# StephenNG59/ICP-symm

Hardware: AMD Instinct MI355X
Metric: icp_iterations_per_sec (higher is better)
Workload: dtype f32

## Files before the change

### icp-symm_amd/csrc/engine_loop.cpp

```cpp
#include "engine_internal.h"

extern "C" {

static int prepare_rejectors(symmicp_ctx *c, RejectArgs &r)
{
    Rejectors &j = c->rej;
    r = RejectArgs{};
    if (!pass_rejects(c)) return SYMMICP_OK;
    HIP_TRY(c, grow(j.keys, j.keys_cap, c->n_loc ? c->n_loc : 1));
    if (!j.ws) HIP_TRY(c, hipMalloc((void **)&j.ws, sizeof(uint32_t) * kRejectWsWords));
    r.keys = j.keys; r.ws = j.ws;
    r.host = reinterpret_cast<RejectRecord *>(c->h_sums_dev + kNSum + 1);
    r.rho = j.trim_frac; r.med_f2 = j.median() ? j.med_factor * j.med_factor : 0.0f;
    if (!pass_claims(c)) return SYMMICP_OK;
    HIP_TRY(c, grow(j.table, j.table_cap, Rejectors::table_words(c->n_t, pass_reciprocal(c))));
    r.table = j.table; r.n_t = c->n_t; r.order = c->src_order;
    r.claim = kClaimOneToOne;
    if (!pass_reciprocal(c)) return SYMMICP_OK;
    if (!j.src_ix.valid) {
        const double t0 = now_s();
        if (int st = build_reverse_index(c, c->src0, c->n_loc, c->src_order, j.src_ix)) return st;
        j.src_ix_builds++;
        if (c->sw.debug_host) {
            std::fprintf(stderr, "[symmicp host] source index: %u points, %zu bytes in its arena (+%zu allocations beside it), built in %.3f ms\n", c->n_loc,
// ... 223 lines not shown
    if (pass_rejects(c)) return false;
    if (c->cfg.mode == SYMMICP_MODE_COLOR) return false;
    if (c->cfg.host_loop) return false;
    if (c->external_exchange || c->shm.slots) return false;
    if (c->timing == 2 || c->ix.dbg) return false;
    if (!mode_device_solves(c->cfg.mode)) return false;
    if (c->n_loc == 0 && !c->comm) return false;
    if (c->host_passes_since_bailout < 2) return false;
    const bool incr = resolved_apply(c->cfg) == SYMMICP_APPLY_INCREMENTAL;
    if (c->cfg.corr == SYMMICP_CORR_IDENTITY) return true;
    if (c->cfg.corr == SYMMICP_CORR_TREE)
        return !incr && c->last_list_len >= 0 && c->last_list_len <= (c->sw.no_loop_stragglers ? 0ll : (long long)kLoopListLimit) && c->last_uncertified >= 0 &&
               c->last_uncertified <= (long long)(loop_scan_limit(c->n_s_total) / (c->last_list_len > 0 ? 2 : 1)) && c->cert && !c->sw.no_cert;
    return false;
}

static constexpr int kListBlocks = 8;
static constexpr int kEvSampleStride = 4;
static int run_batch(symmicp_ctx *c, int want, float *diffs_before, int *n_done, bool *small_step)
{
    *n_done = 0;
    *small_step = false;
    if (want > symmicp_ctx::kRing - 1) want = symmicp_ctx::kRing - 1;
    if (want <= 0) return SYMMICP_OK;
    const bool incr = resolved_apply(c->cfg) == SYMMICP_APPLY_INCREMENTAL;
    const bool tree = c->cfg.corr == SYMMICP_CORR_TREE;
    LoopConfig lc{};
    lc.mode = c->cfg.mode; lc.fixed_iters = c->cfg.fixed_iters; lc.max_iters = c->iters + want; lc.incremental = incr ? 1 : 0; lc.tree = tree ? 1 : 0;
    lc.diff_threshold = c->cfg.diff_threshold; lc.eps_rotation = c->cfg.eps_rotation; lc.eps_translation = c->cfg.eps_translation;
    lc.nrm_w = (c->cfg.mode == SYMMICP_MODE_QUIRKS) ? 1.0f : 0.0f;
    for (int k = 0; k < 3; k++) lc.pivot[k] = c->pivot[k];
    lc.uncertified_limit = 4 * loop_scan_limit(c->n_s_total);
    const bool no_stage = c->sw.no_loop_stragglers;
    bool stragglers = tree && c->last_list_len > 0 && !no_stage;
    lc.list_limit = kLoopListLimit;
    const int cert_mode = (tree && c->cert && !c->sw.no_cert && !c->cert_pass_failed) ? c->sw.cert_pass : 0;
    if (cert_mode == 2) stragglers = false;
    bool cert_chunk = false;
    uint8_t pass_kernel[symmicp_ctx::kRing] = {};
    if (lc.max_iters > c->cfg.max_iters) lc.max_iters = c->cfg.max_iters;
    const int it0 = c->iters;
    const long long list0 = c->last_list_len, scans0 = c->last_scans;
    LoopState ls{};
    std::memcpy(ls.X, c->X, sizeof(ls.X));
    for (int k = 0; k < 12; k++) ls.Xapply.m[k] = c->X[k];
    ls.Xapply.nrm_w = lc.nrm_w;
    ls.iters = it0;
    *c->h_loop = ls;
    symmicp_sums last0{};
    if (c->loop_log_on) {
        last0 = c->last;
        c->h_ring[it0 % symmicp_ctx::kRing].solved = 0;
    }
    HIP_TRY(c, hipMemcpyAsync(c->d_loop, c->h_loop, sizeof(LoopState), hipMemcpyHostToDevice, c->stream));
    PassArgs a{};
    fill_pass_args(c, a, RejectArgs{}, c->X, incr, incr, false);
    a.loop = c->d_loop;
    int blocks;
    bool vec4 = false;
    if (tree) {
        const int fb = c->sw.fused_blocks;
        const int tiles = (int)((c->n_loc + kPassThreads - 1) / kPassThreads);
        blocks = tiles < fb ? tiles : fb;
        if (blocks < 1) blocks = 1;
    } else {
        vec4 = (c->n_loc % 4 == 0) && (c->n_t % 4 == 0) && (c->src_off % 4 == 0);
        const int id_cap = c->sw.id_blocks;
        const int nb = (int)(((vec4 ? c->n_loc / 4 : c->n_loc) + kPassThreads - 1) / kPassThreads);
        blocks = nb < id_cap ? (nb > 0 ? nb : 1) : id_cap;
    }
    const int fused_blocks_full = blocks;
    c->pass_blocks = blocks;
    uint32_t *counters = tree ? c->wl_count : nullptr;
    const bool timed_run = c->timing == 1 || c->timing == 3;
    const int ev_stride = c->timing == 3 ? kEvSampleStride : 1;
    if (timed_run && c->ev_used + want > symmicp_ctx::kEvRing) flush_events(c);
    const bool one_piece = lc.fixed_iters && !(lc.eps_rotation > 0.f && lc.eps_translation > 0.f);
    int enq = 0, n_stage = 0;
    constexpr int kCertHeads = 3;
    int heads_left = (one_piece && !stragglers && cert_mode == 1 && c->sw.cert_head > 0) ? kCertHeads : 0;
    auto plan_chunk = [&](long long list_len, long long scans, int left, int prev) -> int {
        cert_chunk = cert_mode == 2 || (cert_mode == 1 && !stragglers && list_len == 0 && scans == 0);
        if (stragglers) return 4;
        if (!one_piece) return prev ? 2 * prev : 4;
        if (!cert_chunk && heads_left > 0 && left > c->sw.cert_head) { heads_left--; return c->sw.cert_head; }
        return left;
    };
    int chunk = plan_chunk(c->last_list_len, c->last_scans, want, 0);
    bool first_chunk = true;
    while (enq < want) {
        const int nq = (want - enq < chunk) ? want - enq : chunk;
        const int it_before = first_chunk ? it0 : c->h_loop->iters;
        const int ev_used0 = c->ev_used;
        const int fused_blocks = (stragglers && fused_blocks_full + kListBlocks > 512) ? 512 - kListBlocks : fused_blocks_full;
        blocks = fused_blocks + (stragglers ? kListBlocks : 0);
        a.partial_cols = stragglers ? (uint32_t)blocks : 0u;
        a.partial_col0 = (uint32_t)fused_blocks;
        lc.walk_in_loop = stragglers ? 1 : 0;
        if (first_chunk) launch_reduce_solve(c->partials, blocks, c->d_sums, 2, c->d_loop, lc, c->h_ring_dev, symmicp_ctx::kRing, counters, c->stream);
        for (int p = 0; p < nq; p++) {
            hipEvent_t *ev = nullptr;
            if (timed_run && (enq + p) % ev_stride == 0 && c->ev_used < symmicp_ctx::kEvRing) {
                ev = c->ev + c->ev_used * symmicp_ctx::kEvPer;
                c->ev_split[c->ev_used] = 1;
                c->ev_weight[c->ev_used] = 1;
                hipEventRecord(ev[0], c->stream);
            }
            if (tree) {
                pass_kernel[(it_before + 1 + p) % symmicp_ctx::kRing] = cert_chunk ? 1 : 0;
                if (cert_chunk) launch_pass_certified(a, c->ix, c->wl, fused_blocks, c->stream);
                else launch_pass_fused(a, c->ix, c->wl, fused_blocks, c->stream);
                if (stragglers) launch_loop_stragglers(a, c->ix, c->wl, kListBlocks, c->sw.tune, c->stream);
            }
            else launch_pass_identity(a, c->tgt, blocks, vec4, c->stream);
            if (ev) { hipEventRecord(ev[4], c->stream); c->ev_used++; }
            if (c->comm || blocks > 512) {
                launch_final_reduce(c->partials, blocks, c->d_sums, nullptr, c->ticket, 0ull, counters, 0, c->stream);
                if (c->comm) {
                    if (ev) { hipEventRecord(ev[6], c->stream); c->ev_coll[c->ev_used - 1] = 1; }
                    int r = g_rccl.AllReduce(c->d_sums, c->d_sums, kNSum, kNcclFloat64, kNcclSum, c->comm, c->stream);
                    if (r != 0) {
                        (void)hipStreamSynchronize(c->stream);
                        c->begun = false;
                        c->ev_used = 0;
                        return fail(c, SYMMICP_ERR_COMM, std::string("ncclAllReduce: ") + (g_rccl.GetErrorString ? g_rccl.GetErrorString(r) : "?"));
                    }
                    if (ev) hipEventRecord(ev[7], c->stream);
                }
                launch_reduce_solve(c->partials, blocks, c->d_sums, 1, c->d_loop, lc, c->h_ring_dev, symmicp_ctx::kRing, counters, c->stream);
            } else {
                launch_reduce_solve(c->partials, blocks, c->d_sums, 0, c->d_loop, lc, c->h_ring_dev, symmicp_ctx::kRing, counters, c->stream);
            }
        }
        const unsigned long long seq = ++c->batch_seq;
        launch_loop_end(c->d_loop, c->h_loop_dev, c->h_done_dev, seq, c->stream);
        if (int st = wait_for_word(c, c->h_done, seq, 60.0, "batch finished without publishing its end flag")) return st;
        enq += nq;
        first_chunk = false;
        const int ran = (c->h_loop->iters - it_before) + (c->h_loop->reason == LOOP_REDO_PASS ? 1 : 0);
        if (timed_run && ran >= 0) {
            int sampled_ran = 0;
            for (int p = 0; p < ran && p < nq; p++) {
                if ((enq - nq + p) % ev_stride != 0) continue;
                if (ev_used0 + sampled_ran < symmicp_ctx::kEvRing) {
                    const int left = (ran < nq ? ran : nq) - p;
                    c->ev_weight[ev_used0 + sampled_ran] = left < ev_stride ? left : ev_stride;
                }
                sampled_ran++;
            }
            if (ev_used0 + sampled_ran < c->ev_used) c->ev_used = ev_used0 + sampled_ran;
        }
        if (stragglers) n_stage += c->h_loop->iters - it_before;
        if (c->h_loop->stop) break;
        if (tree && !no_stage) {
            stragglers = false;
            for (int k = it_before + 1; k <= c->h_loop->iters; k++) stragglers = stragglers || c->h_ring[k % symmicp_ctx::kRing].list_len > 0;
        }
        if (cert_mode == 2) stragglers = false;
        const LoopRecord &lr = c->h_ring[c->h_loop->iters % symmicp_ctx::kRing];
        chunk = plan_chunk(lr.list_len, lr.reserved, want - enq, chunk);
    }
    const LoopState &hl = *c->h_loop;
    const int it1 = hl.iters;
    if (it1 < it0 || it1 > it0 + want) return fail(c, SYMMICP_ERR_HIP, "device loop state out of range");
    for (int k = it0; k < it1; k++) diffs_before[k - it0] = (k == it0) ? (float)c->last.s[33] : (float)c->h_ring[k % symmicp_ctx::kRing].sums[33];
    if (it1 > it0) {
        std::memcpy(c->last.s, c->h_ring[it1 % symmicp_ctx::kRing].sums, sizeof(double) * kNSum);
        std::memcpy(c->X, c->h_ring[(it1 - 1) % symmicp_ctx::kRing].X, sizeof(float) * 16);
        c->st.passes += it1 - it0;
        c->st.loop_passes += it1 - it0;
        c->st.loop_straggler_passes += n_stage;
    }
    if (c->loop_log_on) {
        for (int k = it0; k <= it1; k++) {
            const LoopRecord &r = c->h_ring[k % symmicp_ctx::kRing];
            symmicp_loop_log_entry e{};
            std::memcpy(e.sums, k == it0 ? last0.s : r.sums, sizeof(e.sums));
            std::memcpy(e.increment, r.increment, sizeof(e.increment));
            std::memcpy(e.X, r.X, sizeof(e.X));
            e.rcond = r.rcond; e.iter = k; e.status = r.status; e.solved = r.solved; e.list_len = k == it0 ? 0 : r.list_len;
            e.reason = hl.reason; e.batch = c->loop_log_batches;
            e.reserved = k == it0 ? 0 : pass_kernel[k % symmicp_ctx::kRing];
            if (k == it1 && hl.reason == LOOP_REDO_PASS && pass_kernel[(it1 + 1) % symmicp_ctx::kRing]) e.reserved |= 0x100;
            if (!e.solved) { std::memset(e.increment, 0, sizeof(e.increment)); std::memset(e.X, 0, sizeof(e.X)); e.rcond = 0.f; e.status = -1; }
            c->loop_log.push_back(e);
        }
        c->loop_log_batches++;
    }
// ... 240 lines not shown
    HIP_TRY(c, hipSetDevice(c->device));
    const size_t b_sums = sizeof(symmicp_sums) * n, b_f3 = sizeof(float) * 3 * n, b_16 = sizeof(float) * 16 * n;
    const size_t o_piv = b_sums, o_xin = o_piv + 16, o_st = o_xin + b_16, o_pb = o_st + 4 * n, o_qb = o_pb + b_f3, o_a = o_qb + b_f3, o_t = o_a + b_f3,
                 o_rc = o_t + b_f3, o_out = o_rc + 4 * n, o_xo = o_out + b_16, total = o_xo + b_16;
    char *d = nullptr;
    HIP_TRY(c, hipMalloc((void **)&d, total));
    float piv[4] = {0.f, 0.f, 0.f, 0.f};
    if (pivot) for (int k = 0; k < 3; k++) piv[k] = pivot[k];
    int st = SYMMICP_OK;
    if (hipMemcpy(d, sums, b_sums, hipMemcpyHostToDevice) != hipSuccess || hipMemcpy(d + o_piv, piv, 16, hipMemcpyHostToDevice) != hipSuccess ||
        (X_in16 && hipMemcpy(d + o_xin, X_in16, b_16, hipMemcpyHostToDevice) != hipSuccess))
        st = fail(c, SYMMICP_ERR_HIP, "probe: upload");
    if (st == SYMMICP_OK) {
        launch_solve_probe(mode, exact_rc, (const symmicp_sums *)d, (int)n, (const float *)(d + o_piv), X_in16 ? (const float *)(d + o_xin) : nullptr,
                           (int32_t *)(d + o_st), (float *)(d + o_pb), (float *)(d + o_qb), (float *)(d + o_a), (float *)(d + o_t), (float *)(d + o_rc),
                           (float *)(d + o_out), (float *)(d + o_xo), c->stream);
        if (hipGetLastError() != hipSuccess || hipStreamSynchronize(c->stream) != hipSuccess) st = fail(c, SYMMICP_ERR_HIP, "probe: kernel");
    }
    if (st == SYMMICP_OK) {
        const struct { size_t off, bytes; void *dst; } back[] = {{o_st, 4 * n, status}, {o_pb, b_f3, pbar}, {o_qb, b_f3, qbar}, {o_a, b_f3, a}, {o_t, b_f3, t},
                                                              {o_rc, 4 * n, rcond}, {o_out, b_16, out16}, {o_xo, X_in16 ? b_16 : 0, X_out16}};
        for (const auto &b : back)
            if (b.bytes && hipMemcpy(b.dst, d + b.off, b.bytes, hipMemcpyDeviceToHost) != hipSuccess) { st = fail(c, SYMMICP_ERR_HIP, "probe: read back"); break; }
    }
    (void)hipFree(d);
    return st;
}

int symmicp_ctx_loop_solve(symmicp_ctx *c, const symmicp_sums *sums, const float pivot[3], const float X_in16[16], const int32_t in_i[6], const float in_f[3],
                           int32_t state_out[4], float X_out16[16], float Xapply_out12[12], float ring_inc16[16], float ring_X16[16], float *ring_rcond,
                           int32_t ring_i2[2])
{
    if (!c) return SYMMICP_ERR_ARG;
    if (!sums || !X_in16 || !in_i || !in_f || !state_out || !X_out16 || !Xapply_out12 || !ring_inc16 || !ring_X16 || !ring_rcond || !ring_i2)
        return fail(c, SYMMICP_ERR_ARG, "loop_solve: bad arguments");
    const int mode = in_i[0];
    if (!mode_device_solves(mode)) return fail(c, SYMMICP_ERR_ARG, "loop_solve: QUIRKS, PAPER, PLANE or GICP");
    HIP_TRY(c, hipSetDevice(c->device));
    LoopConfig lc{};
    lc.mode = mode; lc.fixed_iters = in_i[1]; lc.max_iters = in_i[2]; lc.incremental = in_i[5] ? 1 : 0; lc.tree = 0;
    lc.diff_threshold = in_f[0]; lc.eps_rotation = in_f[1]; lc.eps_translation = in_f[2];
    lc.nrm_w = (mode == SYMMICP_MODE_QUIRKS) ? 1.0f : 0.0f;
    for (int k = 0; k < 3; k++) lc.pivot[k] = pivot ? pivot[k] : 0.f;
    LoopState ls{};
    std::memcpy(ls.X, X_in16, sizeof(ls.X));
    for (int k = 0; k < 12; k++) ls.Xapply.m[k] = X_in16[k];
    ls.Xapply.nrm_w = lc.nrm_w;
    ls.iters = in_i[3];
    ls.small_step = in_i[4];
    char *d = nullptr;
    const size_t o_loop = 512, o_ring = o_loop + ((sizeof(LoopState) + 255) & ~(size_t)255), total = o_ring + sizeof(LoopRecord);
    HIP_TRY(c, hipMalloc((void **)&d, total));
    int st = SYMMICP_OK;
    if (hipMemcpy(d, sums, sizeof(symmicp_sums), hipMemcpyHostToDevice) != hipSuccess || hipMemcpy(d + o_loop, &ls, sizeof(ls), hipMemcpyHostToDevice) != hipSuccess ||
        hipMemset(d + o_ring, 0xFF, sizeof(LoopRecord)) != hipSuccess)
        st = fail(c, SYMMICP_ERR_HIP, "loop_solve: upload");
    if (st == SYMMICP_OK) {
        launch_reduce_solve(nullptr, 0, (double *)d, 2, (LoopState *)(d + o_loop), lc, (LoopRecord *)(d + o_ring), 1, nullptr, c->stream);
        if (hipGetLastError() != hipSuccess || hipStreamSynchronize(c->stream) != hipSuccess) st = fail(c, SYMMICP_ERR_HIP, "loop_solve: kernel");
    }
    LoopState lo{};
    LoopRecord r{};
    if (st == SYMMICP_OK && (hipMemcpy(&lo, d + o_loop, sizeof(lo), hipMemcpyDeviceToHost) != hipSuccess ||
                             hipMemcpy(&r, d + o_ring, sizeof(r), hipMemcpyDeviceToHost) != hipSuccess))
        st = fail(c, SYMMICP_ERR_HIP, "loop_solve: read back");
    (void)hipFree(d);
    if (st != SYMMICP_OK) return st;
    state_out[0] = lo.stop; state_out[1] = lo.reason; state_out[2] = lo.iters; state_out[3] = lo.small_step;
    std::memcpy(X_out16, lo.X, sizeof(lo.X));
    std::memcpy(Xapply_out12, lo.Xapply.m, sizeof(lo.Xapply.m));
    std::memcpy(ring_inc16, r.increment, sizeof(r.increment));
    std::memcpy(ring_X16, r.X, sizeof(r.X));
    std::memcpy(ring_rcond, &r.rcond, sizeof(float));
    ring_i2[0] = r.status; ring_i2[1] = r.solved;
    return SYMMICP_OK;
}

int symmicp_set_loop_log(symmicp_ctx *c, int on)
{
    if (!c) return SYMMICP_ERR_ARG;
    c->loop_log_on = on != 0;
    if (!c->loop_log_on) { c->loop_log.clear(); c->loop_log.shrink_to_fit(); }
    return SYMMICP_OK;
}

int symmicp_get_loop_log(const symmicp_ctx *c, symmicp_loop_log_entry *out, size_t cap, size_t *count)
{
    if (!c || !count) return SYMMICP_ERR_ARG;
    *count = c->loop_log.size();
    if (out) std::memcpy(out, c->loop_log.data(), sizeof(symmicp_loop_log_entry) * std::min(cap, c->loop_log.size()));
    return SYMMICP_OK;
}

}
```

### icp-symm_amd/csrc/kernels_pass.hip

```cpp
#include <cstdlib>
#include <type_traits>
#include "symmicp_internal.h"
#include "device_common.h"
#include "oct_walk.h"
#include "solve_core.h"
#include "robust_loss.h"
#include "pass_rows.h"
#pragma clang fp contract(off)

namespace symmicp {

template <int NA>
__device__ __forceinline__ void acc_block_reduce_store(AccN<NA> &a, double *partials, uint32_t col)
{
    __shared__ double red[(kPassThreads / 64) * kNSum];
    acc_wave_reduce(a, red + (threadIdx.x >> 6) * kNSum);
    __syncthreads();
    if (threadIdx.x < kNSum) {
        double s = 0.0;
        if (threadIdx.x < NA) {
#pragma unroll
            for (int w = 0; w < kPassThreads / 64; w++) s += red[w * kNSum + threadIdx.x];
        }
        partials[(size_t)col * kNSum + threadIdx.x] = s;
// ... 1118 lines not shown

__global__ __launch_bounds__(256) void k_final_reduce(const double *__restrict__ partials, int nblocks,
                                                      double *out_dev, double *out_mapped, uint32_t *ticket,
                                                      unsigned long long seq, uint32_t *counters_to_clear, int keep_nonempty)
{
    __shared__ double red[256];
    const int k = blockIdx.x, t = threadIdx.x;
    double s = 0.0;
    for (int j = t; j < nblocks; j += 256) s += partials[(size_t)j * kNSum + k];
    red[t] = s;
    __syncthreads();
#pragma unroll
    for (int off = 128; off > 0; off >>= 1) {
        if (t < off) red[t] += red[t + off];
        __syncthreads();
    }
    __shared__ int last;
    if (t == 0) {
        out_dev[k] = red[0];
        if (out_mapped) out_mapped[k] = red[0];
        __threadfence_system();
        last = (atomicAdd(ticket, 1u) == gridDim.x - 1);
    }
    __syncthreads();
    if (last) {
        if (counters_to_clear) {
            __shared__ uint32_t s_len;
            if (t < 64) {
                uint32_t len, searched, dropped, scans;
                read_list_words(counters_to_clear, t, len, searched, dropped, scans);
                if (t == 0) {
                    s_len = len;
                    const double lenw = (double)len + (dropped ? kListDropped : 0.0), srw = (double)searched + (double)scans * kScanUnit;
                    out_dev[kNSum - 1] = lenw; out_dev[kNSum - 2] = srw;
                    if (out_mapped) { out_mapped[kNSum - 1] = lenw; out_mapped[kNSum - 2] = srw; }
                }
            }
            __syncthreads();
            if (t < 2) counters_to_clear[t * kShards * kShardStride + 2] = 0;
            if (t < kShards) { counters_to_clear[t * kShardStride + 1] = 0; counters_to_clear[t * kShardStride + 3] = 0; }
            if (!(keep_nonempty && s_len > 0u))
                for (int c = t; c < 2 * kShards; c += 256) counters_to_clear[c * kShardStride] = 0;
        }
        if (t == 0) {
            *ticket = 0;
            if (out_mapped) {
                __threadfence_system();
                reinterpret_cast<volatile unsigned long long *>(out_mapped)[kNSum] = seq;
            }
        }
    }
}

template <bool REDUCE>
__global__ __launch_bounds__(512) void k_reduce_solve(const double *__restrict__ partials, int nblocks, double *out_dev, int solve_only, LoopState *loop,
                                                       LoopConfig cfg, LoopRecord *ring, int ring_len, uint32_t *counters_to_clear)
{
    __shared__ double s_sum[kNSum];
    __shared__ uint32_t s_len, s_unc, s_scan;
    const int t = threadIdx.x, lane = t & 63, wave = t >> 6;
#ifdef RS_STAMPS
    const unsigned long long ts0 = __builtin_amdgcn_s_memrealtime();
#endif
    const LoopState ls = *loop;
    uint32_t cw0 = 0, cw1 = 0, cw2 = 0, cw3 = 0;
    const bool want_counters = !solve_only && REDUCE && counters_to_clear && t < 64;
    if (want_counters) {
        cw0 = counters_to_clear[t * kShardStride]; cw1 = counters_to_clear[t * kShardStride + 1];
        cw2 = (t < 2) ? counters_to_clear[t * kShards * kShardStride + 2] : 0u;
        cw3 = counters_to_clear[t * kShardStride + 3];
    }
    __shared__ double s_part[8][kNSum];
    double accw = 0.0;
    if (!solve_only && REDUCE && lane < kNSum) {
        if (nblocks <= 512) {
            double c[64];
#pragma unroll
            for (int j = 0; j < 64; j++) { const int b = wave + 8 * j; c[j] = (b < nblocks) ? partials[(size_t)b * kNSum + lane] : 0.0; }
#pragma unroll
            for (int j = 0; j < 64; j++) accw += c[j];
        } else {
            for (int b = wave; b < nblocks; b += 8) accw += partials[(size_t)b * kNSum + lane];
        }
    }
    double rec = 0.0;
    if ((solve_only || !REDUCE) && t < kNSum) rec = out_dev[t];
    if (ls.stop) return;
#ifdef RS_STAMPS
    const unsigned long long tsA = __builtin_amdgcn_s_memrealtime();
#endif
    if (t == 0) { s_len = 0; s_unc = 0; s_scan = 0; }
    if (!solve_only && REDUCE) {
        if (lane < kNSum) s_part[wave][lane] = accw;
        __syncthreads();
        if (t < kNSum) {
            double x = 0.0;
#pragma unroll
            for (int w = 0; w < 8; w++) x += s_part[w][t];
            s_sum[t] = (t < kNAccW) ? x : 0.0;
        }
    } else if (t < kNSum) s_sum[t] = rec;
    __syncthreads();
    if (!solve_only && counters_to_clear) {
        if (REDUCE) {
            if (t < 64) {
#pragma unroll
                for (int off = 32; off > 0; off >>= 1) {
                    cw0 += (uint32_t)__shfl_xor((int)cw0, off, 64);
                    cw1 += (uint32_t)__shfl_xor((int)cw1, off, 64);
                    cw2 += (uint32_t)__shfl_xor((int)cw2, off, 64);
                    cw3 += (uint32_t)__shfl_xor((int)cw3, off, 64);
                }
                if (t == 0) { s_len = cw2 ? 0xFFFFFFFFu : cw0; s_unc = cw1; s_scan = cw1 > cw3 ? cw1 - cw3 : 0u; }
            }
            if (t < kShards) { counters_to_clear[t * kShardStride + 1] = 0; counters_to_clear[t * kShardStride + 3] = 0; }
            for (int c = t; c < 2 * kShards; c += 512) counters_to_clear[c * kShardStride] = 0;
        } else if (t == 0) {
            s_len = (s_sum[kNSum - 1] >= kListDropped) ? 0xFFFFFFFFu : (uint32_t)s_sum[kNSum - 1];
            const double sr = s_sum[kNSum - 2], sc = floor(sr / kScanUnit);
            s_unc = (uint32_t)(sr - sc * kScanUnit); s_scan = (uint32_t)sc;
        }
    }
    __syncthreads();
#ifdef RS_STAMPS
    const unsigned long long ts1 = __builtin_amdgcn_s_memrealtime();
#endif
    int it = ls.iters;
    if (!solve_only) {
        const uint32_t len = s_len, unc = s_unc, scans = s_scan;
        if (cfg.tree && len > 0u && (!cfg.walk_in_loop || len == 0xFFFFFFFFu)) { if (t == 0) { loop->stop = 1; loop->reason = LOOP_REDO_PASS; } return; }
        it += 1;
        LoopRecord &r = ring[it % ring_len];
        if (t < kNSum) { const double v = (t >= kNAccW) ? 0.0 : s_sum[t]; r.sums[t] = v; if (REDUCE) out_dev[t] = v; }
        if (t == 0) {
            loop->iters = it;
            r.solved = 0;
            r.pad = (int32_t)unc;
            r.list_len = (int32_t)len; r.reserved = (int32_t)scans;
        }
        if (cfg.tree && (unc > cfg.uncertified_limit || (cfg.walk_in_loop && len > cfg.list_limit))) { if (t == 0) { loop->stop = 1; loop->reason = LOOP_SLOW; } return; }
    }
    if (t != 0) return;
    const float diff = (float)s_sum[33];
    if (ls.small_step || !((cfg.fixed_iters || diff > cfg.diff_threshold) && it < cfg.max_iters)) {
        loop->stop = 1; loop->reason = LOOP_DONE;
        return;
    }
    symmicp_sums S;
    for (int k = 0; k < kNSum; k++) S.s[k] = (k >= kNAccW) ? 0.0 : s_sum[k];
    float pbar[3], qbar[3], av[3], tv[3], rc = 0.f, Xi[16];
    const int st = solve::solve_mode(cfg.mode, S, cfg.pivot, pbar, qbar, av, tv, &rc, Xi, false);
    if (st != SYMMICP_OK || !(rc > 1e-6f)) { loop->stop = 1; loop->reason = LOOP_HOST_SOLVE; return; }
#ifdef RS_STAMPS
    const unsigned long long ts2 = __builtin_amdgcn_s_memrealtime();
#endif
    float Xn[16];
    solve::mat4_mul(Xi, ls.X, Xn);
    for (int k = 0; k < 16; k++) loop->X[k] = Xn[k];
    const float *ap = cfg.incremental ? Xi : Xn;
    for (int k = 0; k < 12; k++) loop->Xapply.m[k] = ap[k];
    loop->Xapply.nrm_w = cfg.nrm_w;
    LoopRecord &r = ring[it % ring_len];
    for (int k = 0; k < 16; k++) { r.increment[k] = Xi[k]; r.X[k] = Xn[k]; }
    r.rcond = rc; r.status = st; r.solved = 1;
#ifdef RS_STAMPS2
    r.sums[37] = partials[(size_t)8191 * kNSum]; r.sums[38] = partials[(size_t)8191 * kNSum + 1]; r.sums[39] = partials[(size_t)8191 * kNSum + 2];
#elif defined(RS_STAMPS)
    r.sums[37] = (double)(ts1 - ts0) + 1e-4 * (double)(tsA - ts0); r.sums[38] = (double)(ts2 - ts1); r.sums[39] = (double)(__builtin_amdgcn_s_memrealtime() - ts2);
#endif
    if (cfg.eps_rotation > 0.f && cfg.eps_translation > 0.f && !cfg.fixed_iters) {
        const double tr = ((double)Xi[0] + Xi[5] + Xi[10] - 1.0) * 0.5;
        const double ang = acos(tr > 1.0 ? 1.0 : (tr < -1.0 ? -1.0 : tr));
        const double tn = sqrt((double)Xi[3] * Xi[3] + (double)Xi[7] * Xi[7] + (double)Xi[11] * Xi[11]);
        if (ang < cfg.eps_rotation && tn < cfg.eps_translation) loop->small_step = 1;
    }
}

__global__ __launch_bounds__(64) void k_solve_probe(int mode, int exact_rc, const symmicp_sums *__restrict__ sums, int n, const float *pivot,
                                                    const float *__restrict__ X_in, int32_t *status, float *pbar, float *qbar, float *a, float *t,
                                                    float *rcond, float *out16, float *X_out)
{
    const int i = blockIdx.x * blockDim.x + threadIdx.x;
    if (i >= n) return;
    const symmicp_sums S = sums[i];
    float pb[3] = {0.f, 0.f, 0.f}, qb[3] = {0.f, 0.f, 0.f}, av[3] = {0.f, 0.f, 0.f}, tv[3] = {0.f, 0.f, 0.f}, rc = 0.f, Xi[16], Xn[16];
    for (int k = 0; k < 16; k++) Xi[k] = 0.f;
    const bool ex = exact_rc != 0;
    const int st = solve::solve_mode(mode, S, pivot, pb, qb, av, tv, &rc, Xi, ex);
    status[i] = st;
    rcond[i] = rc;
    for (int k = 0; k < 3; k++) { pbar[3 * i + k] = pb[k]; qbar[3 * i + k] = qb[k]; a[3 * i + k] = av[k]; t[3 * i + k] = tv[k]; }
    for (int k = 0; k < 16; k++) out16[16 * (size_t)i + k] = Xi[k];
    if (X_in) {
        solve::mat4_mul(Xi, X_in + 16 * (size_t)i, Xn);
        for (int k = 0; k < 16; k++) X_out[16 * (size_t)i + k] = Xn[k];
    }
}

void launch_solve_probe(int mode, int exact_rc, const symmicp_sums *sums, int n, const float *pivot, const float *X_in, int32_t *status, float *pbar,
                        float *qbar, float *a, float *t, float *rcond, float *out16, float *X_out, hipStream_t s)
{
    if (n > 0) hipLaunchKernelGGL(k_solve_probe, dim3((n + 63) / 64), dim3(64), 0, s, mode, exact_rc, sums, n, pivot, X_in, status, pbar, qbar, a, t, rcond, out16, X_out);
}

__global__ __launch_bounds__(64) void k_loop_end(const LoopState *loop, LoopState *host_copy, unsigned long long *done_flag, unsigned long long seq)
{
    if (threadIdx.x == 0) {
        *host_copy = *loop;
        __threadfence_system();
        *reinterpret_cast<volatile unsigned long long *>(done_flag) = seq;
    }
}

__global__ __launch_bounds__(64) void k_publish(const double *__restrict__ sums_dev, double *out_mapped, unsigned long long seq)
{
    if (threadIdx.x < kNSum) out_mapped[threadIdx.x] = sums_dev[threadIdx.x];
    __threadfence_system();
    __syncthreads();
    if (threadIdx.x == 0) {
        __threadfence_system();
        reinterpret_cast<volatile unsigned long long *>(out_mapped)[kNSum] = seq;
    }
}

__global__ __launch_bounds__(kPassThreads) void k_nn_brute(CloudSoA src, uint32_t n_s, Affine X,
                                                          const float4 *__restrict__ tq, uint32_t n_t,
                                                          uint32_t tiles_per_split, unsigned long long *best64)
{
    __shared__ float4 tile[kBruteTile];
    float px[kBruteQ], py[kBruteQ], pz[kBruteQ], bd[kBruteQ];
    uint32_t bj[kBruteQ];
    const uint32_t q0 = blockIdx.x * (kPassThreads * kBruteQ) + threadIdx.x;
#pragma unroll
    for (int k = 0; k < kBruteQ; k++) {
        uint32_t i = q0 + k * kPassThreads;
        float x = 0.f, y = 0.f, z = 0.f;
        if (i < n_s) { x = src.x[i]; y = src.y[i]; z = src.z[i]; }
        px[k] = xf_row(X.m + 0, x, y, z, 1.0f); py[k] = xf_row(X.m + 4, x, y, z, 1.0f); pz[k] = xf_row(X.m + 8, x, y, z, 1.0f);
        bd[k] = __int_as_float(0x7f800000); bj[k] = 0xFFFFFFFFu;
    }
    const uint32_t tile0 = blockIdx.y * tiles_per_split;
    const uint32_t ntiles = (n_t + kBruteTile - 1) / kBruteTile;
    const uint32_t tile1 = min(tile0 + tiles_per_split, ntiles);
    for (uint32_t t = tile0; t < tile1; t++) {
        const uint32_t base = t * kBruteTile;
        __syncthreads();
#pragma unroll
        for (int k = 0; k < kBruteTile / kPassThreads; k++) {
            uint32_t j = base + k * kPassThreads + threadIdx.x;
            tile[k * kPassThreads + threadIdx.x] = (j < n_t) ? tq[j] : make_float4(__int_as_float(0x7fc00000), 0.f, 0.f, 0.f);
        }
        __syncthreads();
#pragma unroll 4
        for (int j = 0; j < kBruteTile; j++) {
            float4 q = tile[j];
#pragma unroll
            for (int k = 0; k < kBruteQ; k++) {
                float d2 = dist2(px[k], py[k], pz[k], q.x, q.y, q.z);
                if (d2 < bd[k]) { bd[k] = d2; bj[k] = base + j; }
            }
        }
    }
#pragma unroll
    for (int k = 0; k < kBruteQ; k++) {
// ... 119 lines not shown
            uint32_t qshift = nb >= 3072u ? 8u : (nb >= 1536u ? 7u : 6u);
            if (tune.cells_queries == 64u) qshift = 6u; else if (tune.cells_queries == 128u) qshift = 7u; else if (tune.cells_queries == 256u) qshift = 8u;
            const uint32_t nq = (a.n + (1u << qshift) - 1u) >> qshift;
            const uint32_t nbc = ((nq + 8u * chunk - 1u) / (8u * chunk)) * (8u * chunk);
            if (a.make_hood) hipLaunchKernelGGL(k_search_cells<true>, dim3(nbc), dim3(kPassThreads), 0, s, a, ix, wl, chunk, qshift);
            else hipLaunchKernelGGL(k_search_cells<false>, dim3(nbc), dim3(kPassThreads), 0, s, a, ix, wl, chunk, qshift);
        }
    }
    if (ev) hipEventRecord(ev[1], s);
    if (ev) hipEventRecord(ev[2], s);
    if (stage != 1 && nbp) {
        if (walk_blocks == 0 || walk_blocks > walk_blocks_full(wl)) walk_blocks = walk_blocks_full(wl);
        const uint32_t wmm = a.pos_prev ? wave_mode_max : 0u;
        if (a.budget_walk) {
            const uint32_t budget = tune.walk_budget;
            hipLaunchKernelGGL(k_search_walk<true>, dim3(walk_blocks), dim3(kWalkThreads), 0, s, a, ix, wl, wl.work, wmm, budget);
            hipLaunchKernelGGL(k_search_walk<false>, dim3(8192), dim3(kWalkThreads), 0, s, a, ix, wl, wl.retry, 0xFFFFFFFFu, 0xFFFFFFFFu);
        } else {
            hipLaunchKernelGGL(k_search_walk<false>, dim3(walk_blocks), dim3(kWalkThreads), 0, s, a, ix, wl, wl.work, wmm, 0xFFFFFFFFu);
        }
    }
    if (ev) hipEventRecord(ev[3], s);
    launch_accumulate(a, ix.tn, acc_blocks, s);
    if (ev) hipEventRecord(ev[4], s);
}

void launch_final_reduce(const double *partials, int blocks, double *out_dev, double *out_host_mapped, uint32_t *ticket,
                         unsigned long long seq, uint32_t *counters_to_clear, int keep_nonempty, hipStream_t s)
{
    hipLaunchKernelGGL(k_final_reduce, dim3(kNSum), dim3(256), 0, s, partials, blocks, out_dev, out_host_mapped, ticket, seq,
                       counters_to_clear, keep_nonempty);
}

void launch_pass_fused(const PassArgs &a, const TargetIndex &ix, const WorkLists &wl, int blocks, hipStream_t s)
{
    with_instantiation(a, [&](auto W, auto OBJ) { hipLaunchKernelGGL((k_pass_fused<true, W, OBJ>), dim3(blocks), dim3(kPassThreads), 0, s, a, ix, wl); });
}

void launch_pass_certified(const PassArgs &a, const TargetIndex &ix, const WorkLists &wl, int blocks, hipStream_t s)
{
    with_instantiation(a, [&](auto W, auto OBJ) { hipLaunchKernelGGL((k_pass_certified<W, OBJ>), dim3(blocks), dim3(kPassThreads), 0, s, a, ix, wl); });
}

void launch_loop_stragglers(const PassArgs &a, const TargetIndex &ix, const WorkLists &wl, int list_blocks, const PassTuning &tune, hipStream_t s)
{
    const uint32_t wave_mode_max = tune.wave_mode_max;
    hipLaunchKernelGGL(k_search_walk<false>, dim3(512), dim3(kWalkThreads), 0, s, a, ix, wl, wl.work, wave_mode_max, 0xFFFFFFFFu);
    with_instantiation(a, [&](auto W, auto OBJ) {
        hipLaunchKernelGGL((k_accumulate_list<W, OBJ>), dim3(list_blocks), dim3(kPassThreads), 0, s, a, ix.tn, wl.work);
    });
}

void launch_reduce_solve(const double *partials, int blocks, double *out_dev, int mode, LoopState *loop, LoopConfig cfg, LoopRecord *ring, int ring_len,
                         uint32_t *counters_to_clear, hipStream_t s)
{
    if (mode == 0) hipLaunchKernelGGL(k_reduce_solve<true>, dim3(1), dim3(512), 0, s, partials, blocks, out_dev, 0, loop, cfg, ring, ring_len, counters_to_clear);
    else hipLaunchKernelGGL(k_reduce_solve<false>, dim3(1), dim3(512), 0, s, partials, blocks, out_dev, mode == 2 ? 1 : 0, loop, cfg, ring, ring_len, counters_to_clear);
}

void launch_loop_end(const LoopState *loop, LoopState *host_copy, unsigned long long *done_flag, unsigned long long seq, hipStream_t s)
{
    hipLaunchKernelGGL(k_loop_end, dim3(1), dim3(64), 0, s, loop, host_copy, done_flag, seq);
}

void launch_publish(const double *sums_dev, double *out_host_mapped, unsigned long long seq, hipStream_t s)
{
    hipLaunchKernelGGL(k_publish, dim3(1), dim3(64), 0, s, sums_dev, out_host_mapped, seq);
}

void launch_nn_brute(const CloudSoA &src, uint32_t n_s, const Affine &X, const float4 *tq, uint32_t n_t,
                     unsigned long long *best64, hipStream_t s)
{
    const uint32_t qblocks = (n_s + kPassThreads * kBruteQ - 1) / (kPassThreads * kBruteQ);
    const uint32_t ntiles = (n_t + kBruteTile - 1) / kBruteTile;
    uint32_t splits = 1;
    if (qblocks < 2048) splits = (2048 + qblocks - 1) / qblocks;
    if (splits > ntiles) splits = ntiles;
    if (splits < 1) splits = 1;
    if (splits > 65535) splits = 65535;
    const uint32_t tiles_per_split = (ntiles + splits - 1) / splits;
    splits = (ntiles + tiles_per_split - 1) / tiles_per_split;
    hipMemsetAsync(best64, 0xFF, sizeof(unsigned long long) * (size_t)n_s, s);
    hipLaunchKernelGGL(k_nn_brute, dim3(qblocks, splits), dim3(kPassThreads), 0, s, src, n_s, X, tq, n_t, tiles_per_split, best64);
}

}
```

### icp-symm_amd/csrc/symmicp_internal.h

```cpp
#pragma once
#include <hip/hip_runtime.h>
#include <stdint.h>
#include <stddef.h>
#include "symmicp.h"

namespace symmicp {

constexpr int kNSum = SYMMICP_NSUM;
constexpr int kNAcc = 37;
constexpr int kNAccW = 38;
constexpr double kListDropped = 4294967296.0;
constexpr double kScanUnit = 4294967296.0;
constexpr int kLeaf = 8;
constexpr int kFan = 8;
constexpr int kMaxTreeLevels = 12;
constexpr int kMortonBits = 10;
constexpr int kPassThreads = 256;
constexpr int kBruteTile = 1024;
constexpr int kBruteQ = 4;

constexpr bool mode_device_solves(int mode)
{
    return mode == SYMMICP_MODE_QUIRKS || mode == SYMMICP_MODE_PAPER || mode == SYMMICP_MODE_PLANE || mode == SYMMICP_MODE_GICP;
}
// ... 147 lines not shown
    RejectArgs rej;
    const float4 *tgt_color;
    const float *src_int;
    float color_lam, color_om;
};
static_assert(sizeof(PassArgs) == 432 && offsetof(PassArgs, rej) == 344 && offsetof(PassArgs, tgt_color) == 408 && offsetof(PassArgs, src_int) == 416,
              "PassArgs keeps its layout");
__host__ __device__ inline bool pass_rejects(const PassArgs &a) { return a.rej.keys != nullptr; }

struct PassTuning {
    uint32_t wave_mode_max = 20000u;
    uint32_t cells_chunk = 16u;
    uint32_t cells_queries = 0u;
    uint32_t walk_budget = 160u;
};

constexpr int kBatchThreads = 512;
constexpr int kBatchQ = 4;
constexpr int kBatchChunk = kBatchThreads * kBatchQ;
constexpr int kBatchTile = SYMMICP_BATCH_MAX_POINTS;
constexpr int kBatchMerge = 1024;
__host__ __device__ constexpr uint32_t batch_splits(uint32_t n) { return n <= 256u ? 8u : n <= 512u ? 4u : n <= 1024u ? 2u : 1u; }
static_assert(kBatchThreads / 8 >= 64 && (kBatchThreads / 2) * kBatchQ == kBatchMerge, "a split is at least one wave; two splits cover kBatchMerge rows");
struct BatchProblem {
    uint32_t src_first, src_count, tgt_first, tgt_count;
    float pivot[3];
    uint32_t slot;
};
struct BatchArgs {
    const float *src_xyz, *src_nrm, *tgt_xyz, *tgt_nrm;
    const BatchProblem *problems;
    const float *guess;
    symmicp_batch_result *out;
    float *trace_X;
    double *trace_sums;
    int32_t mode, max_iters, fixed_iters;
    float diff_threshold, max_d2, min_ndot, eps_rotation, eps_translation;
};
void launch_batch_align(const BatchArgs &a, uint32_t n_problems, hipStream_t s);

void launch_pass_identity(const PassArgs &a, CloudSoA tgt, int blocks, bool vec4_ok, hipStream_t s);
void launch_pass_indexed(const PassArgs &a, const float4 *tn , int blocks, hipStream_t s);
void launch_pass_tree_split(const PassArgs &a, const TargetIndex &ix, const WorkLists &wl, int acc_blocks, uint32_t walk_blocks,
                            int stage, int compact_blocks, const PassTuning &tune, hipStream_t s, hipEvent_t *ev);
void launch_pass_tree_first(const PassArgs &a, const TargetIndex &ix, const WorkLists &wl, int acc_blocks, hipStream_t s, hipEvent_t *ev);
uint32_t walk_blocks_full(const WorkLists &wl);
uint32_t shard_capacity(uint32_t n_points);
void launch_final_reduce(const double *partials, int blocks, double *out_dev, double *out_host_mapped, uint32_t *ticket,
                         unsigned long long seq, uint32_t *counters_to_clear, int keep_nonempty, hipStream_t s);
void launch_pass_fused(const PassArgs &a, const TargetIndex &ix, const WorkLists &wl, int blocks, hipStream_t s);
void launch_pass_certified(const PassArgs &a, const TargetIndex &ix, const WorkLists &wl, int blocks, hipStream_t s);
void launch_loop_stragglers(const PassArgs &a, const TargetIndex &ix, const WorkLists &wl, int list_blocks, const PassTuning &tune, hipStream_t s);
void launch_reduce_solve(const double *partials, int blocks, double *out_dev, int mode, LoopState *loop, LoopConfig cfg, LoopRecord *ring, int ring_len,
                         uint32_t *counters_to_clear, hipStream_t s);
void launch_solve_probe(int mode, int exact_rc, const symmicp_sums *sums, int n, const float *pivot, const float *X_in, int32_t *status, float *pbar,
                        float *qbar, float *a, float *t, float *rcond, float *out16, float *X_out, hipStream_t s);
void launch_loop_end(const LoopState *loop, LoopState *host_copy, unsigned long long *done_flag, unsigned long long seq, hipStream_t s);
void launch_publish(const double *sums_dev, double *out_host_mapped, unsigned long long seq, hipStream_t s);
void launch_nn_brute(const CloudSoA &src, uint32_t n_s, const Affine &X, const float4 *tq, uint32_t n_t,
                     unsigned long long *best64, hipStream_t s);

void launch_bbox(const float *x, const float *y, const float *z, uint32_t n, uint32_t *bbox_ord6, hipStream_t s);
void launch_morton(const float *x, const float *y, const float *z, uint32_t n, float ox, float oy, float oz,
                   float inv_h0, uint32_t *keys, uint32_t *vals, hipStream_t s);
void radix_sort_pairs(uint32_t *keys, uint32_t *vals, uint32_t *keys_tmp, uint32_t *vals_tmp, uint32_t n,
                      int key_bits, uint32_t *hist_ws, size_t hist_ws_elems, hipStream_t s);
size_t radix_sort_ws_elems(uint32_t n);
void launch_gather_f4(const float *x, const float *y, const float *z, const float *nx, const float *ny, const float *nz,
                      const uint32_t *order, uint32_t n, float4 *tq, float4 *tn, hipStream_t s);
void launch_gather_soa(const CloudSoA &src, const uint32_t *order, uint32_t n, CloudSoA dst, hipStream_t s);
void launch_offset_u32(const uint32_t *in, uint32_t off, uint32_t n, uint32_t *out, hipStream_t s);
void launch_packet_runs(const CloudSoA &src, uint32_t n, float jump_factor, uint2 *runs, uint32_t *keys, uint32_t *vals, uint32_t *count, int key_bits, hipStream_t s);
void launch_packet_cost(const CloudSoA &src, const uint2 *runs, uint32_t npk, const TargetIndex &ix, uint32_t *keys, int key_bits, hipStream_t s);
void launch_packet_table(const uint32_t *order, const uint2 *runs, uint32_t npk, uint2 *tab, hipStream_t s);
void launch_deinterleave3(const float *raw, size_t row_stride, size_t offset, uint32_t n, float *x, float *y, float *z, hipStream_t s);
void launch_level_hist(const uint32_t *keys, uint32_t n, uint32_t *hist16, hipStream_t s);
void launch_cell_table(const uint32_t *keys, uint32_t n, int glevel, const uint32_t *nid_top, uint32_t *ctop, uint2 *cells, hipStream_t s);
void launch_oct_flags(const uint32_t *keys, uint32_t n, int level, uint32_t *nid, hipStream_t s);
void launch_exclusive_scan(uint32_t *data, uint32_t n, uint32_t *tile_ws , hipStream_t s);
void launch_oct_first(const uint32_t *keys, uint32_t n, int level, const uint32_t *nid, uint32_t *first, hipStream_t s);
void launch_oct_nodes(int level, const float4 *tq, uint32_t n, const uint32_t *first, uint32_t n_nodes, const uint32_t *nid_next,
                      uint32_t n_nodes_next, const float4 *nodes_next, float4 *nodes, uint32_t leaf_max, hipStream_t s);
void launch_leaf_boxes(const float4 *tq, uint32_t n, float4 *boxes, uint32_t nleaf_padded, hipStream_t s);
void launch_node_boxes(const float4 *child, uint32_t nchild_padded, float4 *parent, uint32_t nparent_padded, hipStream_t s);
void launch_iota_f4(const float *x, const float *y, const float *z, const float *nx, const float *ny, const float *nz,
                    uint32_t n, float4 *tq, float4 *tn, hipStream_t s);
void launch_unpermute(const CloudSoA &cur, const uint32_t *order, uint32_t n, float *xyz_aos, float *nrm_aos, hipStream_t s);
void launch_corr_out(const int32_t *pos, const unsigned long long *best64, const float *d2, const float4 *tq,
                     const uint32_t *src_order, uint32_t n, int mode, uint32_t tgt_offset, int32_t *idx_out, float *d2_out,
                     const uint32_t *rej_keys , uint32_t rej_tau, hipStream_t s);

void launch_reject(const PassArgs &a, int corr, CloudSoA tgt, const float4 *tn, hipStream_t s);
void launch_select_probe(const uint32_t *keys, uint32_t n, uint32_t k, uint32_t *ws, hipStream_t s);
void launch_unique_probe(const int32_t *tgt_row, const uint32_t *d2_bits, uint32_t n, unsigned long long *table, uint32_t n_t,
                         uint8_t *winner_out, hipStream_t s);

void launch_relabel_tq(float4 *tq, uint32_t n, const uint32_t *labels, hipStream_t s);
void launch_reverse_nn_probe(const TargetIndex &six, const Affine &inv, const float *q_xyz, uint32_t n_q, int32_t *label_out, float *d2_out, hipStream_t s);

void launch_identity_d2(const CloudSoA &in, const Affine &X, const CloudSoA &tgt, uint32_t tgt_offset, uint32_t n, float *d2, hipStream_t s);
void launch_pairs_d2(const CloudSoA &in, const Affine &X, const int32_t *pos, const float4 *tq, uint32_t n_t, uint32_t n, float *d2, hipStream_t s);
void launch_normals_knn(const TargetIndex &ix, int k, const float vp[3], float *nrm_out, float *curv_out, hipStream_t s);
void launch_knn(const TargetIndex &ix, int k, int32_t *rows_out, float *d2_out, hipStream_t s);

void launch_color_permute_target(const float *intensity, const float *grad3, const float4 *tq, uint32_t n, float4 *dst, hipStream_t s);
void launch_color_permute_source(const float *intensity, const uint32_t *order, uint32_t off, uint32_t n, float *dst, hipStream_t s);
void launch_color_unpermute_source(const float *src_int, const uint32_t *order, uint32_t n, float *out_rows, hipStream_t s);
void launch_color_gradient(const TargetIndex &ix, const float *intensity_rows, const int32_t *knn_rows, int k, float4 *rec_rows, float *grad_rows,
                           hipStream_t s);

// ... 83 lines not shown
```

Measured before the change: 33260.

## Fold loop-end publish and initial state upload into reduce-solve kernel

Removes the separate loop-end kernel by having the last reduce-solve launch of each batch write the loop state to host-mapped memory and set the done flag. It also drops the host-to-device memcpy of the initial loop state, passing it as a kernel argument to the first solve-only launch instead. The solve kernel now builds the final state in shared memory and writes it out one word per lane from a single wave. This saves a kernel launch and a copy per batch, at the cost of a larger kernel argument and more complex control flow in the solve kernel.

```diff
diff --git a/icp-symm_amd/csrc/engine_loop.cpp b/icp-symm_amd/csrc/engine_loop.cpp
--- a/icp-symm_amd/csrc/engine_loop.cpp
+++ b/icp-symm_amd/csrc/engine_loop.cpp
@@ -299,7 +299,6 @@
         last0 = c->last;
         c->h_ring[it0 % symmicp_ctx::kRing].solved = 0;
     }
-    HIP_TRY(c, hipMemcpyAsync(c->d_loop, c->h_loop, sizeof(LoopState), hipMemcpyHostToDevice, c->stream));
     PassArgs a{};
     fill_pass_args(c, a, RejectArgs{}, c->X, incr, incr, false);
     a.loop = c->d_loop;
@@ -344,8 +343,10 @@
         a.partial_cols = stragglers ? (uint32_t)blocks : 0u;
         a.partial_col0 = (uint32_t)fused_blocks;
         lc.walk_in_loop = stragglers ? 1 : 0;
-        if (first_chunk) launch_reduce_solve(c->partials, blocks, c->d_sums, 2, c->d_loop, lc, c->h_ring_dev, symmicp_ctx::kRing, counters, c->stream);
+        if (first_chunk) launch_reduce_solve(c->partials, blocks, c->d_sums, 2, c->d_loop, lc, c->h_ring_dev, symmicp_ctx::kRing, counters, &ls, nullptr, nullptr, 0ull, c->stream);
+        const unsigned long long seq = ++c->batch_seq;
         for (int p = 0; p < nq; p++) {
+            const bool last = p == nq - 1;
             hipEvent_t *ev = nullptr;
             if (timed_run && (enq + p) % ev_stride == 0 && c->ev_used < symmicp_ctx::kEvRing) {
                 ev = c->ev + c->ev_used * symmicp_ctx::kEvPer;
@@ -374,13 +375,13 @@
                     }
                     if (ev) hipEventRecord(ev[7], c->stream);
                 }
-                launch_reduce_solve(c->partials, blocks, c->d_sums, 1, c->d_loop, lc, c->h_ring_dev, symmicp_ctx::kRing, counters, c->stream);
+                launch_reduce_solve(c->partials, blocks, c->d_sums, 1, c->d_loop, lc, c->h_ring_dev, symmicp_ctx::kRing, counters, nullptr, last ? c->h_loop_dev : nullptr,
+                                    last ? c->h_done_dev : nullptr, last ? seq : 0ull, c->stream);
             } else {
-                launch_reduce_solve(c->partials, blocks, c->d_sums, 0, c->d_loop, lc, c->h_ring_dev, symmicp_ctx::kRing, counters, c->stream);
+                launch_reduce_solve(c->partials, blocks, c->d_sums, 0, c->d_loop, lc, c->h_ring_dev, symmicp_ctx::kRing, counters, nullptr, last ? c->h_loop_dev : nullptr,
+                                    last ? c->h_done_dev : nullptr, last ? seq : 0ull, c->stream);
             }
         }
-        const unsigned long long seq = ++c->batch_seq;
-        launch_loop_end(c->d_loop, c->h_loop_dev, c->h_done_dev, seq, c->stream);
         if (int st = wait_for_word(c, c->h_done, seq, 60.0, "batch finished without publishing its end flag")) return st;
         enq += nq;
         first_chunk = false;
@@ -727,11 +728,11 @@
     const size_t o_loop = 512, o_ring = o_loop + ((sizeof(LoopState) + 255) & ~(size_t)255), total = o_ring + sizeof(LoopRecord);
     HIP_TRY(c, hipMalloc((void **)&d, total));
     int st = SYMMICP_OK;
-    if (hipMemcpy(d, sums, sizeof(symmicp_sums), hipMemcpyHostToDevice) != hipSuccess || hipMemcpy(d + o_loop, &ls, sizeof(ls), hipMemcpyHostToDevice) != hipSuccess ||
+    if (hipMemcpy(d, sums, sizeof(symmicp_sums), hipMemcpyHostToDevice) != hipSuccess || hipMemset(d + o_loop, 0xFF, sizeof(LoopState)) != hipSuccess ||
         hipMemset(d + o_ring, 0xFF, sizeof(LoopRecord)) != hipSuccess)
         st = fail(c, SYMMICP_ERR_HIP, "loop_solve: upload");
     if (st == SYMMICP_OK) {
-        launch_reduce_solve(nullptr, 0, (double *)d, 2, (LoopState *)(d + o_loop), lc, (LoopRecord *)(d + o_ring), 1, nullptr, c->stream);
+        launch_reduce_solve(nullptr, 0, (double *)d, 2, (LoopState *)(d + o_loop), lc, (LoopRecord *)(d + o_ring), 1, nullptr, &ls, nullptr, nullptr, 0ull, c->stream);
         if (hipGetLastError() != hipSuccess || hipStreamSynchronize(c->stream) != hipSuccess) st = fail(c, SYMMICP_ERR_HIP, "loop_solve: kernel");
     }
     LoopState lo{};
diff --git a/icp-symm_amd/csrc/kernels_pass.hip b/icp-symm_amd/csrc/kernels_pass.hip
--- a/icp-symm_amd/csrc/kernels_pass.hip
+++ b/icp-symm_amd/csrc/kernels_pass.hip
@@ -1194,17 +1194,56 @@
     }
 }
 
-template <bool REDUCE>
-__global__ __launch_bounds__(512) void k_reduce_solve(const double *__restrict__ partials, int nblocks, double *out_dev, int solve_only, LoopState *loop,
-                                                       LoopConfig cfg, LoopRecord *ring, int ring_len, uint32_t *counters_to_clear)
+struct LoopPublish {
+    LoopState *host_copy;
+    unsigned long long *done_flag;
+    unsigned long long seq;
+};
+struct NoLoopEntry {};
+constexpr int kLoopWords = (int)(sizeof(LoopState) / sizeof(uint32_t));
+static_assert(sizeof(LoopState) % sizeof(uint32_t) == 0 && kLoopWords <= 64, "the loop state is written out one word per lane of one wave");
+
+__device__ __forceinline__ void wave_lds_sync()
+{
+    __builtin_amdgcn_fence(__ATOMIC_RELEASE, "wavefront");
+    __builtin_amdgcn_wave_barrier();
+    __builtin_amdgcn_fence(__ATOMIC_ACQUIRE, "wavefront");
+}
+
+__device__ __forceinline__ void loop_state_out(const LoopState &fin, LoopState *loop, bool to_dev, const LoopPublish &pub, int lane)
+{
+    wave_lds_sync();
+    if (lane < kLoopWords) {
+        const uint32_t v = reinterpret_cast<const uint32_t *>(&fin)[lane];
+        if (to_dev) reinterpret_cast<uint32_t *>(loop)[lane] = v;
+        if (pub.host_copy) reinterpret_cast<uint32_t *>(pub.host_copy)[lane] = v;
+    }
+    if (pub.host_copy) {
+        __threadfence_system();
+        if (lane == 0) *reinterpret_cast<volatile unsigned long long *>(pub.done_flag) = pub.seq;
+    }
+}
+
+template <bool REDUCE, bool SOLVE_ONLY>
+__global__ __launch_bounds__(512) void k_reduce_solve(const double *__restrict__ partials, int nblocks, double *out_dev, LoopState *loop,
+                                                       LoopConfig cfg, LoopRecord *ring, int ring_len, uint32_t *counters_to_clear, LoopPublish pub,
+                                                       std::conditional_t<SOLVE_ONLY, LoopState, NoLoopEntry> entry)
 {
     __shared__ double s_sum[kNSum];
     __shared__ uint32_t s_len, s_unc, s_scan;
+    __shared__ LoopState s_fin;
+    constexpr bool solve_only = SOLVE_ONLY;
     const int t = threadIdx.x, lane = t & 63, wave = t >> 6;
 #ifdef RS_STAMPS
     const unsigned long long ts0 = __builtin_amdgcn_s_memrealtime();
 #endif
-    const LoopState ls = *loop;
+    LoopState ls;
+    uint32_t lsw = 0;
+    if constexpr (SOLVE_ONLY) ls = entry;
+    else {
+        ls = *loop;
+        if (t < kLoopWords) lsw = reinterpret_cast<const uint32_t *>(loop)[t];
+    }
     uint32_t cw0 = 0, cw1 = 0, cw2 = 0, cw3 = 0;
     const bool want_counters = !solve_only && REDUCE && counters_to_clear && t < 64;
     if (want_counters) {
@@ -1227,7 +1266,12 @@
     }
     double rec = 0.0;
     if ((solve_only || !REDUCE) && t < kNSum) rec = out_dev[t];
-    if (ls.stop) return;
+    if constexpr (SOLVE_ONLY) { if (t == 0) s_fin = ls; }
+    else if (t < kLoopWords) reinterpret_cast<uint32_t *>(&s_fin)[t] = lsw;
+    if (ls.stop) {
+        if (wave == 0 && (SOLVE_ONLY || pub.host_copy)) loop_state_out(s_fin, loop, SOLVE_ONLY, pub, lane);
+        return;
+    }
 #ifdef RS_STAMPS
     const unsigned long long tsA = __builtin_amdgcn_s_memrealtime();
 #endif
@@ -1267,55 +1311,66 @@
 #ifdef RS_STAMPS
     const unsigned long long ts1 = __builtin_amdgcn_s_memrealtime();
 #endif
+    if (wave != 0) return;
     int it = ls.iters;
+    int reason = LOOP_RUNNING;
     if (!solve_only) {
         const uint32_t len = s_len, unc = s_unc, scans = s_scan;
-        if (cfg.tree && len > 0u && (!cfg.walk_in_loop || len == 0xFFFFFFFFu)) { if (t == 0) { loop->stop = 1; loop->reason = LOOP_REDO_PASS; } return; }
-        it += 1;
-        LoopRecord &r = ring[it % ring_len];
-        if (t < kNSum) { const double v = (t >= kNAccW) ? 0.0 : s_sum[t]; r.sums[t] = v; if (REDUCE) out_dev[t] = v; }
-        if (t == 0) {
-            loop->iters = it;
-            r.solved = 0;
-            r.pad = (int32_t)unc;
-            r.list_len = (int32_t)len; r.reserved = (int32_t)scans;
-        }
-        if (cfg.tree && (unc > cfg.uncertified_limit || (cfg.walk_in_loop && len > cfg.list_limit))) { if (t == 0) { loop->stop = 1; loop->reason = LOOP_SLOW; } return; }
-    }
-    if (t != 0) return;
-    const float diff = (float)s_sum[33];
-    if (ls.small_step || !((cfg.fixed_iters || diff > cfg.diff_threshold) && it < cfg.max_iters)) {
-        loop->stop = 1; loop->reason = LOOP_DONE;
-        return;
-    }
-    symmicp_sums S;
-    for (int k = 0; k < kNSum; k++) S.s[k] = (k >= kNAccW) ? 0.0 : s_sum[k];
-    float pbar[3], qbar[3], av[3], tv[3], rc = 0.f, Xi[16];
-    const int st = solve::solve_mode(cfg.mode, S, cfg.pivot, pbar, qbar, av, tv, &rc, Xi, false);
-    if (st != SYMMICP_OK || !(rc > 1e-6f)) { loop->stop = 1; loop->reason = LOOP_HOST_SOLVE; return; }
+        if (cfg.tree && len > 0u && (!cfg.walk_in_loop || len == 0xFFFFFFFFu)) reason = LOOP_REDO_PASS;
+        else {
+            it += 1;
+            LoopRecord &r = ring[it % ring_len];
+            if (t < kNSum) { const double v = (t >= kNAccW) ? 0.0 : s_sum[t]; r.sums[t] = v; if (REDUCE) out_dev[t] = v; }
+            if (t == 0) {
+                s_fin.iters = it;
+                r.solved = 0;
+                r.pad = (int32_t)unc;
+                r.list_len = (int32_t)len; r.reserved = (int32_t)scans;
+            }
+            if (cfg.tree && (unc > cfg.uncertified_limit || (cfg.walk_in_loop && len > cfg.list_limit))) reason = LOOP_SLOW;
+        }
+    }
+    if (reason == LOOP_RUNNING) {
+        const float diff = (float)s_sum[33];
+        if (ls.small_step || !((cfg.fixed_iters || diff > cfg.diff_threshold) && it < cfg.max_iters)) reason = LOOP_DONE;
+    }
 #ifdef RS_STAMPS
-    const unsigned long long ts2 = __builtin_amdgcn_s_memrealtime();
+    unsigned long long ts2 = ts1;
 #endif
-    float Xn[16];
-    solve::mat4_mul(Xi, ls.X, Xn);
-    for (int k = 0; k < 16; k++) loop->X[k] = Xn[k];
-    const float *ap = cfg.incremental ? Xi : Xn;
-    for (int k = 0; k < 12; k++) loop->Xapply.m[k] = ap[k];
-    loop->Xapply.nrm_w = cfg.nrm_w;
-    LoopRecord &r = ring[it % ring_len];
-    for (int k = 0; k < 16; k++) { r.increment[k] = Xi[k]; r.X[k] = Xn[k]; }
-    r.rcond = rc; r.status = st; r.solved = 1;
+    if (reason == LOOP_RUNNING && lane == 0) {
+        symmicp_sums S;
+        for (int k = 0; k < kNSum; k++) S.s[k] = (k >= kNAccW) ? 0.0 : s_sum[k];
+        float pbar[3], qbar[3], av[3], tv[3], rc = 0.f, Xi[16];
+        const int st = solve::solve_mode(cfg.mode, S, cfg.pivot, pbar, qbar, av, tv, &rc, Xi, false);
+        if (st != SYMMICP_OK || !(rc > 1e-6f)) reason = LOOP_HOST_SOLVE;
+        else {
+#ifdef RS_STAMPS
+            ts2 = __builtin_amdgcn_s_memrealtime();
+#endif
+            float Xn[16];
+            solve::mat4_mul(Xi, ls.X, Xn);
+            for (int k = 0; k < 16; k++) s_fin.X[k] = Xn[k];
+            const float *ap = cfg.incremental ? Xi : Xn;
+            for (int k = 0; k < 12; k++) s_fin.Xapply.m[k] = ap[k];
+            s_fin.Xapply.nrm_w = cfg.nrm_w;
+            LoopRecord &r = ring[it % ring_len];
+            for (int k = 0; k < 16; k++) { r.increment[k] = Xi[k]; r.X[k] = Xn[k]; }
+            r.rcond = rc; r.status = st; r.solved = 1;
 #ifdef RS_STAMPS2
-    r.sums[37] = partials[(size_t)8191 * kNSum]; r.sums[38] = partials[(size_t)8191 * kNSum + 1]; r.sums[39] = partials[(size_t)8191 * kNSum + 2];
+            r.sums[37] = partials[(size_t)8191 * kNSum]; r.sums[38] = partials[(size_t)8191 * kNSum + 1]; r.sums[39] = partials[(size_t)8191 * kNSum + 2];
 #elif defined(RS_STAMPS)
-    r.sums[37] = (double)(ts1 - ts0) + 1e-4 * (double)(tsA - ts0); r.sums[38] = (double)(ts2 - ts1); r.sums[39] = (double)(__builtin_amdgcn_s_memrealtime() - ts2);
+            r.sums[37] = (double)(ts1 - ts0) + 1e-4 * (double)(tsA - ts0); r.sums[38] = (double)(ts2 - ts1); r.sums[39] = (double)(__builtin_amdgcn_s_memrealtime() - ts2);
 #endif
-    if (cfg.eps_rotation > 0.f && cfg.eps_translation > 0.f && !cfg.fixed_iters) {
-        const double tr = ((double)Xi[0] + Xi[5] + Xi[10] - 1.0) * 0.5;
-        const double ang = acos(tr > 1.0 ? 1.0 : (tr < -1.0 ? -1.0 : tr));
-        const double tn = sqrt((double)Xi[3] * Xi[3] + (double)Xi[7] * Xi[7] + (double)Xi[11] * Xi[11]);
-        if (ang < cfg.eps_rotation && tn < cfg.eps_translation) loop->small_step = 1;
-    }
+            if (cfg.eps_rotation > 0.f && cfg.eps_translation > 0.f && !cfg.fixed_iters) {
+                const double tr = ((double)Xi[0] + Xi[5] + Xi[10] - 1.0) * 0.5;
+                const double ang = acos(tr > 1.0 ? 1.0 : (tr < -1.0 ? -1.0 : tr));
+                const double tn = sqrt((double)Xi[3] * Xi[3] + (double)Xi[7] * Xi[7] + (double)Xi[11] * Xi[11]);
+                if (ang < cfg.eps_rotation && tn < cfg.eps_translation) s_fin.small_step = 1;
+            }
+        }
+    }
+    if (reason != LOOP_RUNNING && lane == 0) { s_fin.stop = 1; s_fin.reason = reason; }
+    loop_state_out(s_fin, loop, true, pub, lane);
 }
 
 __global__ __launch_bounds__(64) void k_solve_probe(int mode, int exact_rc, const symmicp_sums *__restrict__ sums, int n, const float *pivot,
@@ -1343,15 +1398,6 @@
                         float *qbar, float *a, float *t, float *rcond, float *out16, float *X_out, hipStream_t s)
 {
     if (n > 0) hipLaunchKernelGGL(k_solve_probe, dim3((n + 63) / 64), dim3(64), 0, s, mode, exact_rc, sums, n, pivot, X_in, status, pbar, qbar, a, t, rcond, out16, X_out);
-}
-
-__global__ __launch_bounds__(64) void k_loop_end(const LoopState *loop, LoopState *host_copy, unsigned long long *done_flag, unsigned long long seq)
-{
-    if (threadIdx.x == 0) {
-        *host_copy = *loop;
-        __threadfence_system();
-        *reinterpret_cast<volatile unsigned long long *>(done_flag) = seq;
-    }
 }
 
 __global__ __launch_bounds__(64) void k_publish(const double *__restrict__ sums_dev, double *out_mapped, unsigned long long seq)
@@ -1577,15 +1623,13 @@
 }
 
 void launch_reduce_solve(const double *partials, int blocks, double *out_dev, int mode, LoopState *loop, LoopConfig cfg, LoopRecord *ring, int ring_len,
-                         uint32_t *counters_to_clear, hipStream_t s)
-{
-    if (mode == 0) hipLaunchKernelGGL(k_reduce_solve<true>, dim3(1), dim3(512), 0, s, partials, blocks, out_dev, 0, loop, cfg, ring, ring_len, counters_to_clear);
-    else hipLaunchKernelGGL(k_reduce_solve<false>, dim3(1), dim3(512), 0, s, partials, blocks, out_dev, mode == 2 ? 1 : 0, loop, cfg, ring, ring_len, counters_to_clear);
-}
-
-void launch_loop_end(const LoopState *loop, LoopState *host_copy, unsigned long long *done_flag, unsigned long long seq, hipStream_t s)
-{
-    hipLaunchKernelGGL(k_loop_end, dim3(1), dim3(64), 0, s, loop, host_copy, done_flag, seq);
+                         uint32_t *counters_to_clear, const LoopState *entry, LoopState *host_copy, unsigned long long *done_flag, unsigned long long seq,
+                         hipStream_t s)
+{
+    const LoopPublish pub{host_copy, done_flag, seq};
+    if (mode == 0) hipLaunchKernelGGL((k_reduce_solve<true, false>), dim3(1), dim3(512), 0, s, partials, blocks, out_dev, loop, cfg, ring, ring_len, counters_to_clear, pub, NoLoopEntry{});
+    else if (mode == 1) hipLaunchKernelGGL((k_reduce_solve<false, false>), dim3(1), dim3(512), 0, s, partials, blocks, out_dev, loop, cfg, ring, ring_len, counters_to_clear, pub, NoLoopEntry{});
+    else hipLaunchKernelGGL((k_reduce_solve<false, true>), dim3(1), dim3(512), 0, s, partials, blocks, out_dev, loop, cfg, ring, ring_len, counters_to_clear, pub, *entry);
 }
 
 void launch_publish(const double *sums_dev, double *out_host_mapped, unsigned long long seq, hipStream_t s)
diff --git a/icp-symm_amd/csrc/symmicp_internal.h b/icp-symm_amd/csrc/symmicp_internal.h
--- a/icp-symm_amd/csrc/symmicp_internal.h
+++ b/icp-symm_amd/csrc/symmicp_internal.h
@@ -223,10 +223,10 @@
 void launch_pass_certified(const PassArgs &a, const TargetIndex &ix, const WorkLists &wl, int blocks, hipStream_t s);
 void launch_loop_stragglers(const PassArgs &a, const TargetIndex &ix, const WorkLists &wl, int list_blocks, const PassTuning &tune, hipStream_t s);
 void launch_reduce_solve(const double *partials, int blocks, double *out_dev, int mode, LoopState *loop, LoopConfig cfg, LoopRecord *ring, int ring_len,
-                         uint32_t *counters_to_clear, hipStream_t s);
+                         uint32_t *counters_to_clear, const LoopState *entry, LoopState *host_copy, unsigned long long *done_flag, unsigned long long seq,
+                         hipStream_t s);
 void launch_solve_probe(int mode, int exact_rc, const symmicp_sums *sums, int n, const float *pivot, const float *X_in, int32_t *status, float *pbar,
                         float *qbar, float *a, float *t, float *rcond, float *out16, float *X_out, hipStream_t s);
-void launch_loop_end(const LoopState *loop, LoopState *host_copy, unsigned long long *done_flag, unsigned long long seq, hipStream_t s);
 void launch_publish(const double *sums_dev, double *out_host_mapped, unsigned long long seq, hipStream_t s);
 void launch_nn_brute(const CloudSoA &src, uint32_t n_s, const Affine &X, const float4 *tq, uint32_t n_t,
                      unsigned long long *best64, hipStream_t s);
```

After: 33410, median of 5. Within noise of the previous version (+0.5%).
